# mapbox/robosat

Hardware: NVIDIA H100
Metric: 512x512 tiles/sec (predict fwd) (higher is better)
Workload: dtype f16 hi+lo operand pairs (3 MMAs per K step), fp32 accumulate: strict precision, meets the parity contract

## Files before the change

robosat_b200/csrc/rsb_conv.cu:

```cuda

#include <stdio.h>
#include <string.h>

#include <new>

#include "../../include/rsb200.h"
#include "rsb_host.h"
#include "rsb_ptx.cuh"

namespace rsb {

static constexpr int kBlockM = 128;
static constexpr int kBlockK = 64;
static constexpr int kABytes = kBlockM * kBlockK * 2;
static constexpr int kWgRows = 64;

struct alignas(64) ConvKParams {
    CUtensorMap tmA[RSB_MAX_SRCS];
    CUtensorMap tmB;
    CUtensorMap tmC[4];
    CUtensorMap tmR;
    int32_t nseg;
    int32_t seg_src[RSB_MAX_SEGS];
    int32_t seg_dh[RSB_MAX_SEGS];
    int32_t seg_dw[RSB_MAX_SEGS];
    int32_t seg_cb[RSB_MAX_SEGS];
    int32_t kblocks;
    int32_t tiles_w, tiles_h, tiles_n, n_blocks, phases, total_tiles;
    int32_t pair_tiles;
    int32_t TW, TH, TN;
    int32_t Wt, Ht, Nt;
    int32_t Cout;
    int32_t out_sy, out_sx;
    int64_t out_pitch_w, out_pitch_h, out_pitch_n;
    __half* out;
    const __half* residual;
    const float* bias;
    int32_t relu;
    int32_t head_classes;
    const float* head_w;
    const float* head_b;
    float* head_out;
    float acc_scale;
    float* stats;
    int32_t kchunk;
    float* scratch;
};

template <int BLOCK_N, int MODE, bool HAS_RES, bool TWO = false, int SPLIT = 0>
struct ConvCfg {
    static_assert(SPLIT != 2 || (BLOCK_N <= 64 && !TWO), "the N-concatenated split schedule is for narrow single-CTA tiles");
    static constexpr int kAccN = SPLIT == 2 ? 2 * BLOCK_N : BLOCK_N;
    static constexpr int kPlanes = SPLIT ? 2 : 1;
    static constexpr int kBBytes = BLOCK_N * kBlockK * 2;
    static constexpr int kBHalf = kBBytes / 2;
    static constexpr int kStageA = kPlanes * kABytes;
    static constexpr int kStageB = kPlanes * kBBytes;
    static constexpr int kStageBytes = kStageA + kStageB;
    static constexpr int kChunk = BLOCK_N >= 64 ? 64 : 32;
    static constexpr int kNumChunks = BLOCK_N / kChunk;
    static constexpr int kThreads = 384;
    static constexpr int kWgChunkBytes = kWgRows * kChunk * 2;
    static constexpr int kSliceBytes = kPlanes * kWgChunkBytes;
    static constexpr int kStoreBufs = SPLIT ? 1 : 2;
    static constexpr int kResBufs = HAS_RES ? 2 : 0;
    static constexpr int kEpiBytes = MODE == 0 ? (kStoreBufs + kResBufs) * 2 * kSliceBytes : 0;
    static constexpr int kBarBytes = 512;
    static constexpr int kMaxSmem = 232448;
    static constexpr int kAvail = kMaxSmem - 1024 - kBarBytes - kEpiBytes;
    static constexpr int kStages = (kAvail / kStageBytes) > 8 ? 8 : (kAvail / kStageBytes);
    static_assert(kStages >= 2, "pipeline too shallow");
    static constexpr int kSmemBytes = kStages * kStageBytes + kEpiBytes + kBarBytes + 1024;
};

struct TileCoord {
    int n_blk, pa, pb, phase, w0, h0, n0;
};

__device__ __forceinline__ TileCoord decode_tile(const ConvKParams& p, int id) {
    TileCoord t;
    t.n_blk = id % p.n_blocks;
    id /= p.n_blocks;
    t.phase = id % p.phases;
    id /= p.phases;
    t.pa = t.phase >> 1;
    t.pb = t.phase & 1;
    t.w0 = (id % p.tiles_w) * p.TW;
    id /= p.tiles_w;
    t.h0 = (id % p.tiles_h) * p.TH;
    id /= p.tiles_h;
    t.n0 = id * p.TN;
    return t;
}

template <bool TWO>
__device__ __forceinline__ int item_tile(const ConvKParams& p, int it, int rank) {
    if (!TWO) return it;
    const int per = p.n_blocks * p.phases;
    return ((it / per) * 2 + rank) * per + it % per;
}

__device__ __forceinline__ bool row_valid(const ConvKParams& p, const TileCoord& t, int row) {
    const int w = t.w0 + row % p.TW, h = t.h0 + (row / p.TW) % p.TH, n = t.n0 + row / (p.TW * p.TH);
    return (w < p.Wt) && (h < p.Ht) && (n < p.Nt);
}

template <int BLOCK_N, int MODE, bool HAS_RES, bool TWO, int SPLIT, bool STATS = false>
__global__ void __launch_bounds__(384, 1) conv_tc_kernel(const __grid_constant__ ConvKParams p) {
    using Cfg = ConvCfg<BLOCK_N, MODE, HAS_RES, TWO, SPLIT>;
    const int rank = TWO ? static_cast<int>(cluster_ctarank()) : 0;
    const int item0 = TWO ? static_cast<int>(blockIdx.x >> 1) : static_cast<int>(blockIdx.x);
    const int item_step = TWO ? static_cast<int>(gridDim.x >> 1) : static_cast<int>(gridDim.x);
    const int num_items = TWO ? p.pair_tiles : p.total_tiles;
    extern __shared__ uint8_t smem_raw[];
    uint8_t* smem = reinterpret_cast<uint8_t*>((reinterpret_cast<uintptr_t>(smem_raw) + 1023) & ~uintptr_t(1023));
    uint8_t* smem_a = smem;
    uint8_t* smem_b = smem + Cfg::kStages * Cfg::kStageA;
    uint8_t* smem_c = smem + Cfg::kStages * Cfg::kStageBytes;
    uint8_t* smem_r = smem_c + Cfg::kStoreBufs * 2 * Cfg::kSliceBytes;
    uint64_t* full_bar = reinterpret_cast<uint64_t*>(smem + Cfg::kStages * Cfg::kStageBytes + Cfg::kEpiBytes);
    uint64_t* empty_bar = full_bar + Cfg::kStages;
    uint64_t* res_full_bar = empty_bar + Cfg::kStages;

    const int warp_idx = threadIdx.x >> 5;
    const int lane = threadIdx.x & 31;

    if (warp_idx == 8 && lane == 0) {
        for (int i = 0; i < RSB_MAX_SRCS; ++i) tma_prefetch_desc(&p.tmA[i]);
        tma_prefetch_desc(&p.tmB);
        for (int i = 0; i < Cfg::kStages; ++i) {
            mbar_init(&full_bar[i], 1);
            mbar_init(&empty_bar[i], (TWO ? 2 : 1) * 8);
        }
        for (int i = 0; i < 4; ++i) mbar_init(&res_full_bar[i], 1);
        if (MODE == 0) {
            for (int i = 0; i < 4; ++i) tma_prefetch_desc(&p.tmC[i]);
            if (HAS_RES) tma_prefetch_desc(&p.tmR);
        }
        mbar_fence_init();
    }
    if (TWO) cluster_sync_all();
    else __syncthreads();

    asm volatile("griddepcontrol.launch_dependents;" ::: "memory");
    asm volatile("griddepcontrol.wait;" ::: "memory");

    if (warp_idx >= 8) {
        setmaxnreg_dec<40>();
        if (warp_idx == 8 && elect_one()) {
            int stage = 0;
            uint32_t phase = 0;
            for (int it = item0; it < num_items; it += item_step) {
                const TileCoord t = decode_tile(p, item_tile<TWO>(p, it, rank));
                const int b_row = t.phase * p.Cout + t.n_blk * BLOCK_N;
                int kb = 0;
                for (int s = 0; s < p.nseg; ++s) {
                    const CUtensorMap* tm = &p.tmA[p.seg_src[s]];
                    const int cw = t.w0 + p.seg_dw[s] + t.pb;
                    const int ch = t.h0 + p.seg_dh[s] + t.pa;
                    for (int cb = 0; cb < p.seg_cb[s]; ++cb, ++kb) {
                        mbar_wait(&empty_bar[stage], phase ^ 1);
                        mbar_expect_tx(&full_bar[stage], Cfg::kStageBytes);
                        uint8_t* sa = smem_a + stage * Cfg::kStageA;
                        uint8_t* sb = smem_b + stage * Cfg::kStageB;
                        if constexpr (SPLIT) {
                            tma_load_5d(sa, tm, &full_bar[stage], cb * kBlockK, cw, ch, t.n0, 0);
                        } else {
                            tma_load_4d(sa, tm, &full_bar[stage], cb * kBlockK, cw, ch, t.n0);
                        }
                        if constexpr (TWO) {
                            const int hrow = b_row + rank * (BLOCK_N / 2);
                            if constexpr (SPLIT) {
                                tma_load_3d_mc(sb + rank * Cfg::kBHalf, &p.tmB, &full_bar[stage], kb * kBlockK, hrow, 0, 3);
                                tma_load_3d_mc(sb + Cfg::kBBytes + rank * Cfg::kBHalf, &p.tmB, &full_bar[stage], kb * kBlockK, hrow, 1, 3);
                            } else {
                                tma_load_2d_mc(sb + rank * Cfg::kBHalf, &p.tmB, &full_bar[stage], kb * kBlockK, hrow, 3);
                            }
                        } else if constexpr (SPLIT) {
                            tma_load_3d(sb, &p.tmB, &full_bar[stage], kb * kBlockK, b_row, 0);
                        } else {
                            tma_load_2d(sb, &p.tmB, &full_bar[stage], kb * kBlockK, b_row);
                        }
                        if (++stage == Cfg::kStages) {
                            stage = 0;
                            phase ^= 1;
                        }
                    }
                }
            }
        }
    } else {
        setmaxnreg_inc<232>();
        const int g = warp_idx >> 2;
        const int wtid = threadIdx.x & 127;
        const int r0 = 16 * (warp_idx & 3) + (lane >> 2);
        const int cq = 2 * (lane & 3);
        const int qrow0 = g * kWgRows;
        const int qw = qrow0 % p.TW, qh = (qrow0 / p.TW) % p.TH, qn = qrow0 / (p.TW * p.TH);
        uint8_t* my_c = smem_c + g * Cfg::kStoreBufs * Cfg::kSliceBytes;
        uint8_t* my_r = smem_r + g * (Cfg::kResBufs > 0 ? Cfg::kResBufs : 1) * Cfg::kSliceBytes;
        uint64_t* my_res_bar = res_full_bar + g * 2;
        const uint32_t peer_empty0 = TWO ? mapa_u32(smem_u32(&empty_bar[0]), rank ^ 1) : 0;
        auto release_stage = [&](int s) {
            __syncwarp();
            if (lane == 0) {
                mbar_arrive(&empty_bar[s]);
                if (TWO) mbar_arrive_remote(peer_empty0 + s * 8);
            }
        };
        uint32_t wchunk = 0;
        int res_item = item0;
        int res_chunk = 0;
        auto issue_residual = [&](int rb) {
            if (res_item < num_items) {
                const TileCoord rt = decode_tile(p, item_tile<TWO>(p, res_item, rank));
                mbar_expect_tx(&my_res_bar[rb], Cfg::kSliceBytes);
                if constexpr (SPLIT)
                    tma_load_5d(my_r + rb * Cfg::kSliceBytes, &p.tmR, &my_res_bar[rb], rt.n_blk * BLOCK_N + res_chunk * Cfg::kChunk,
                                rt.w0 + qw, rt.h0 + qh, rt.n0 + qn, 0);
                else
                    tma_load_4d(my_r + rb * Cfg::kSliceBytes, &p.tmR, &my_res_bar[rb], rt.n_blk * BLOCK_N + res_chunk * Cfg::kChunk,
                                rt.w0 + qw, rt.h0 + qh, rt.n0 + qn);
                if (++res_chunk == Cfg::kNumChunks) {
                    res_chunk = 0;
                    res_item += item_step;
                }
            }
        };
        if (MODE == 0 && HAS_RES && wtid == 0) {
#pragma unroll 1
            for (int i = 0; i < Cfg::kResBufs; ++i) issue_residual(i);
        }
        const uint64_t da0 = make_sw128_kmajor_desc(smem_u32(smem_a + g * kWgRows * 128));
        const uint64_t db0 = make_sw128_kmajor_desc(smem_u32(smem_b));
        int stage = 0;
        uint32_t phase = 0;
        const int kchunk = p.kchunk > 0 ? p.kchunk : p.kblocks;
        const int nchunks = (p.kblocks + kchunk - 1) / kchunk;
        float acc[Cfg::kAccN / 2];

        for (int it = item0; it < num_items; it += item_step) {
            const TileCoord t = decode_tile(p, item_tile<TWO>(p, it, rank));
            float* srow0 = p.scratch + (static_cast<size_t>(blockIdx.x) * kBlockM + qrow0 + r0) * BLOCK_N;
            for (int chk = 0; chk < nchunks; ++chk) {
                const int kb0 = chk * kchunk;
                const int kb1 = kb0 + kchunk < p.kblocks ? kb0 + kchunk : p.kblocks;
                int prev = -1;
                for (int kb = kb0; kb < kb1; ++kb) {
                    mbar_wait(&full_bar[stage], phase);
                    const uint64_t da = da0 + static_cast<uint64_t>(stage * (Cfg::kStageA >> 4));
                    const uint64_t db = db0 + static_cast<uint64_t>(stage * (Cfg::kStageB >> 4));
                    acc_fence(acc);
                    wgmma_fence();
#pragma unroll
                    for (int k = 0; k < kBlockK / 16; ++k) {
                        const uint32_t first = (kb != kb0 || k != 0) ? 1u : 0u;
                        if constexpr (SPLIT == 2) {
                            wgmma<2 * BLOCK_N>(acc, da + 2 * k, db + 2 * k, first);
                            wgmma<BLOCK_N, BLOCK_N / 2>(acc, da + (kABytes >> 4) + 2 * k, db + 2 * k, 1u);
                        } else if constexpr (SPLIT == 1) {
                            const uint64_t dal = da + (kABytes >> 4), dbl = db + (Cfg::kBBytes >> 4);
                            wgmma<BLOCK_N>(acc, da + 2 * k, dbl + 2 * k, first);
                            wgmma<BLOCK_N>(acc, dal + 2 * k, db + 2 * k, 1u);
                            wgmma<BLOCK_N>(acc, da + 2 * k, db + 2 * k, 1u);
                        } else {
                            wgmma<BLOCK_N>(acc, da + 2 * k, db + 2 * k, first);
                        }
                    }
                    wgmma_commit();
                    acc_fence(acc);
                    wgmma_wait<1>();
                    if (prev >= 0) release_stage(prev);
                    prev = stage;
                    if (++stage == Cfg::kStages) {
                        stage = 0;
                        phase ^= 1;
                    }
                }
                wgmma_wait<0>();
                acc_fence(acc);
                release_stage(prev);
                if (BLOCK_N <= 128 && nchunks > 1) {
                    const bool last = chk + 1 == nchunks;
#pragma unroll
                    for (int j = 0; j < BLOCK_N / 8; ++j) {
#pragma unroll
                        for (int hh = 0; hh < 2; ++hh) {
                            float* sp = srow0 + hh * 8 * BLOCK_N + 8 * j + cq;
                            const int i = 4 * j + 2 * hh;
                            if constexpr (SPLIT == 2) {
                                acc[i] += acc[BLOCK_N / 2 + i];
                                acc[i + 1] += acc[BLOCK_N / 2 + i + 1];
                                acc[BLOCK_N / 2 + i] = 0.f;
                                acc[BLOCK_N / 2 + i + 1] = 0.f;
                            }
                            if (chk > 0) {
                                const float2 o = *reinterpret_cast<const float2*>(sp);
                                acc[i] += o.x;
                                acc[i + 1] += o.y;
                            }
                            if (!last) *reinterpret_cast<float2*>(sp) = make_float2(acc[i], acc[i + 1]);
                        }
                    }
                }
            }
            auto accv = [&](int j, int hh, int e) {
                float v = acc[4 * j + 2 * hh + e];
                if constexpr (SPLIT == 2) v += acc[BLOCK_N / 2 + 4 * j + 2 * hh + e];
                return v;
            };

            if constexpr (MODE == 0) {
                const float* bptr = p.bias ? p.bias + t.n_blk * BLOCK_N : nullptr;
                const float asc = p.acc_scale;
#pragma unroll
                for (int ck = 0; ck < Cfg::kNumChunks; ++ck, ++wchunk) {
                    constexpr int kRB = Cfg::kResBufs > 0 ? Cfg::kResBufs : 1;
                    const int rb = wchunk % kRB;
                    uint8_t* cbuf = my_c + (wchunk % Cfg::kStoreBufs) * Cfg::kSliceBytes;
                    const uint8_t* rbuf = my_r + rb * Cfg::kSliceBytes;
                    if (wtid == 0) tma_store_wait_read<Cfg::kStoreBufs - 1>();
                    named_bar_sync(1 + g, 128);
                    if (HAS_RES) mbar_wait(&my_res_bar[rb], (wchunk / kRB) & 1);
#pragma unroll
                    for (int jj = 0; jj < Cfg::kChunk / 8; ++jj) {
                        const int j = ck * (Cfg::kChunk / 8) + jj;
                        const int c = 8 * j + cq;
                        float2 b2 = make_float2(0.f, 0.f);
                        if (bptr) b2 = __ldg(reinterpret_cast<const float2*>(bptr + c));
#pragma unroll
                        for (int hh = 0; hh < 2; ++hh) {
                            const int r = r0 + 8 * hh;
                            const int su = Cfg::kChunk == 64 ? (jj ^ (r & 7)) : (jj ^ ((r >> 1) & 3));
                            const int soff = r * (Cfg::kChunk * 2) + su * 16 + (lane & 3) * 4;
                            float a = bptr ? fmaf(accv(j, hh, 0), asc, b2.x) : accv(j, hh, 0) * asc;
                            float b = bptr ? fmaf(accv(j, hh, 1), asc, b2.y) : accv(j, hh, 1) * asc;
                            if (HAS_RES) {
                                const float2 f = __half22float2(*reinterpret_cast<const __half2*>(rbuf + soff));
                                if constexpr (SPLIT) {
                                    const float2 l = __half22float2(*reinterpret_cast<const __half2*>(rbuf + Cfg::kWgChunkBytes + soff));
                                    a += f.x + l.x;
                                    b += f.y + l.y;
                                } else {
                                    a += f.x;
                                    b += f.y;
                                }
                            }
                            if (p.relu) {
                                a = fmaxf(a, 0.0f);
                                b = fmaxf(b, 0.0f);
                            }
                            const __half2 o = __floats2half2_rn(a, b);
                            *reinterpret_cast<__half2*>(cbuf + soff) = o;
                            if constexpr (SPLIT) {
                                const float2 hf = __half22float2(o);
                                *reinterpret_cast<__half2*>(cbuf + Cfg::kWgChunkBytes + soff) = __floats2half2_rn(a - hf.x, b - hf.y);
                            }
                        }
                    }
                    fence_proxy_async_smem();
                    named_bar_sync(1 + g, 128);
                    if constexpr (STATS) {
                        const int hq = warp_idx & 3;
                        if (hq < 2) {
                            const unsigned vmask = __ballot_sync(0xffffffffu, row_valid(p, t, qrow0 + 32 * hq + lane));
                            constexpr int kWords = Cfg::kChunk / 2;
                            constexpr int kGroups = 32 / kWords;
                            const int wd = lane % kWords, gr = lane / kWords;
                            float s0x = 0.f, s0y = 0.f, s1x = 0.f, s1y = 0.f;
#pragma unroll 8
                            for (int r = gr; r < 32; r += kGroups) {
                                const int rr = 32 * hq + r;
                                const int u = wd >> 2;
                                const int su = Cfg::kChunk == 64 ? (u ^ (rr & 7)) : (u ^ ((rr >> 1) & 3));
                                const __half2 hv = *reinterpret_cast<const __half2*>(cbuf + rr * (Cfg::kChunk * 2) + su * 16 + (wd & 3) * 4);
                                if ((vmask >> r) & 1u) {
                                    const float2 f = __half22float2(hv);
                                    s0x += f.x;
                                    s0y += f.y;
                                    s1x = fmaf(f.x, f.x, s1x);
                                    s1y = fmaf(f.y, f.y, s1y);
                                }
                            }
                            if (kGroups == 2) {
                                s0x += __shfl_xor_sync(0xffffffffu, s0x, 16);
                                s0y += __shfl_xor_sync(0xffffffffu, s0y, 16);
                                s1x += __shfl_xor_sync(0xffffffffu, s1x, 16);
                                s1y += __shfl_xor_sync(0xffffffffu, s1y, 16);
                            }
                            const int spatial = item_tile<TWO>(p, it, rank) / p.n_blocks;
                            if (gr == 0 && spatial < p.tiles_w * p.tiles_h * p.tiles_n) {
                                const int q = 2 * g + hq;
                                float* dst = p.stats + (static_cast<size_t>(spatial) * 4 + q) * 2 * p.Cout + t.n_blk * BLOCK_N + ck * Cfg::kChunk + 2 * wd;
                                *reinterpret_cast<float2*>(dst) = make_float2(s0x, s0y);
                                *reinterpret_cast<float2*>(dst + p.Cout) = make_float2(s1x, s1y);
                            }
                        }
                    }
                    if (wtid == 0) {
                        if constexpr (SPLIT)
                            tma_store_5d(&p.tmC[t.phase], cbuf, t.n_blk * BLOCK_N + ck * Cfg::kChunk, t.w0 + qw, t.h0 + qh, t.n0 + qn, 0);
                        else
                            tma_store_4d(&p.tmC[t.phase], cbuf, t.n_blk * BLOCK_N + ck * Cfg::kChunk, t.w0 + qw, t.h0 + qh, t.n0 + qn);
                        tma_store_commit();
                        if (HAS_RES) issue_residual(rb);
                    }
                }
            } else {
                static_assert(MODE == 0 || BLOCK_N == 32, "head mode needs BLOCK_N == 32");
#pragma unroll
                for (int hh = 0; hh < 2; ++hh) {
                    const int row = qrow0 + r0 + 8 * hh;
                    float v[8];
#pragma unroll
                    for (int j = 0; j < 4; ++j) {
#pragma unroll
                        for (int e = 0; e < 2; ++e) {
                            float a = accv(j, hh, e) * p.acc_scale;
                            if (p.bias) a += __ldg(p.bias + 8 * j + cq + e);
                            v[2 * j + e] = p.relu ? fmaxf(a, 0.0f) : a;
                        }
                    }
                    const bool valid = row_valid(p, t, row);
                    const int w = t.w0 + row % p.TW, h = t.h0 + (row / p.TW) % p.TH, n = t.n0 + row / (p.TW * p.TH);
                    for (int k = 0; k < p.head_classes; ++k) {
                        float s = 0.f;
#pragma unroll
                        for (int j = 0; j < 4; ++j) {
                            s = fmaf(__ldg(p.head_w + k * 32 + 8 * j + cq), v[2 * j], s);
                            s = fmaf(__ldg(p.head_w + k * 32 + 8 * j + cq + 1), v[2 * j + 1], s);
                        }
                        s += __shfl_xor_sync(0xffffffffu, s, 1);
                        s += __shfl_xor_sync(0xffffffffu, s, 2);
                        if (valid && (lane & 3) == 0) p.head_out[((static_cast<int64_t>(n) * p.head_classes + k) * p.Ht + h) * p.Wt + w] = s + __ldg(p.head_b + k);
                    }
                }
            }
        }
        if (MODE == 0 && wtid == 0) tma_store_wait<0>();
    }

    if (TWO) cluster_sync_all();
}

__global__ void conv_simt_check_kernel(rsb_conv_desc d, int K) {
    const int64_t total_px = static_cast<int64_t>(d.Nt) * d.Ht * d.Wt * d.phases;
    const int co_per_thread = d.mode == 1 ? d.Cout : 1;
    const int co_threads = d.Cout / co_per_thread;
    const int64_t gid = static_cast<int64_t>(blockIdx.x) * blockDim.x + threadIdx.x;
    if (gid >= total_px * co_threads) return;
    const int co0 = static_cast<int>(gid % co_threads) * co_per_thread;
    int64_t px = gid / co_threads;
    const int phase = static_cast<int>(px % d.phases);
    px /= d.phases;
    const int w = static_cast<int>(px % d.Wt);
    px /= d.Wt;
    const int h = static_cast<int>(px % d.Ht);
    const int n = static_cast<int>(px / d.Ht);
    const int pa = phase >> 1, pb = phase & 1;
    const __half* wts = static_cast<const __half*>(d.weights);
    const int64_t w_plane = static_cast<int64_t>(d.phases) * d.Cout * K;

    float head_acc[8];
    for (int k = 0; k < 8; ++k) head_acc[k] = (d.mode == 1 && k < d.head_classes) ? d.head_b[k] : 0.f;

    for (int co = co0; co < co0 + co_per_thread; ++co) {
        const __half* wrow = wts + (static_cast<int64_t>(phase) * d.Cout + co) * K;
        float acc = 0.f;
        int kidx = 0;
        for (int s = 0; s < d.nseg; ++s) {
            const rsb_conv_src& src = d.srcs[d.segs[s].src];
            const int hh = h + d.segs[s].dh + pa, ww = w + d.segs[s].dw + pb;
            const bool inb = hh >= 0 && hh < src.H && ww >= 0 && ww < src.W && n < src.N;
            const __half* a = static_cast<const __half*>(src.ptr) + n * src.pitch_n + hh * src.pitch_h + ww * src.pitch_w;
            for (int c = 0; c < d.segs[s].cblocks * 64; ++c, ++kidx) {
                if (inb && c < src.C) {
                    float av = __half2float(a[c]), wv = __half2float(wrow[kidx]);
                    if (d.split) {
                        av += __half2float(a[c + src.plane]);
                        wv += __half2float(wrow[kidx + w_plane]);
                    }
                    acc = fmaf(av, wv, acc);
                }
            }
        }
        acc *= d.acc_scale != 0.f ? d.acc_scale : 1.f;
        if (d.bias) acc += d.bias[co];
        const int64_t off = n * d.out_pitch_n + static_cast<int64_t>(h * d.out_sy + pa) * d.out_pitch_h +
                            static_cast<int64_t>(w * d.out_sx + pb) * d.out_pitch_w + co;
        if (d.mode == 0) {
            if (d.residual) {
                float rv = __half2float(static_cast<const __half*>(d.residual)[off]);
                if (d.split) rv += __half2float(static_cast<const __half*>(d.residual)[off + d.res_plane]);
                acc += rv;
            }
            if (d.relu) acc = fmaxf(acc, 0.f);
            const __half hi = __float2half_rn(acc);
            static_cast<__half*>(d.out)[off] = hi;
            if (d.split) static_cast<__half*>(d.out)[off + d.out_plane] = __float2half_rn(acc - __half2float(hi));
        } else {
            if (d.relu) acc = fmaxf(acc, 0.f);
            for (int k = 0; k < d.head_classes; ++k) head_acc[k] = fmaf(d.head_w[k * 32 + co], acc, head_acc[k]);
        }
    }
    if (d.mode == 1) {
        for (int k = 0; k < d.head_classes; ++k)
            d.head_out[((static_cast<int64_t>(n) * d.head_classes + k) * d.Ht + h) * d.Wt + w] = head_acc[k];
    }
}

}

using namespace rsb;

struct rsb_conv_plan {
    ConvKParams kp;
    int block_n;
    int mode;
    int grid;
    int smem;
    bool has_res;
    bool pair;
    bool split;
    bool stats;
};

static int validate_desc(const rsb_conv_desc* d, int* K_out) {
    if (!d) return set_error(RSB_E_INVALID, "conv: null desc");
    if (d->nsrc < 1 || d->nsrc > RSB_MAX_SRCS) return set_error(RSB_E_INVALID, "conv: nsrc out of range");
    if (d->nseg < 1 || d->nseg > RSB_MAX_SEGS) return set_error(RSB_E_INVALID, "conv: nseg out of range");
    if (!(d->block_n == 32 || d->block_n == 64 || d->block_n == 128 || d->block_n == 256))
        return set_error(RSB_E_INVALID, "conv: block_n must be 32/64/128/256");
    if (d->Cout <= 0 || d->Cout % d->block_n) return set_error(RSB_E_INVALID, "conv: Cout not a multiple of block_n");
    if (!(d->phases == 1 || d->phases == 4)) return set_error(RSB_E_INVALID, "conv: phases must be 1 or 4");
    if (d->TW * d->TH * d->TN != kBlockM) return set_error(RSB_E_INVALID, "conv: TW*TH*TN must be 128");
    if (d->Wt <= 0 || d->Ht <= 0 || d->Nt <= 0) return set_error(RSB_E_INVALID, "conv: empty tile space");
    if (!d->weights) return set_error(RSB_E_INVALID, "conv: null weights");
    if (d->split != 0 && d->split != 1) return set_error(RSB_E_INVALID, "conv: split must be 0 or 1");
    int kblocks = 0;
    for (int s = 0; s < d->nseg; ++s) {
        const rsb_conv_seg& g = d->segs[s];
        if (g.src < 0 || g.src >= d->nsrc || g.cblocks < 1) return set_error(RSB_E_INVALID, "conv: bad segment");
        if (g.cblocks * kBlockK > ((d->srcs[g.src].C + kBlockK - 1) / kBlockK) * kBlockK)
            return set_error(RSB_E_INVALID, "conv: segment reads past the source's inner extent");
        kblocks += g.cblocks;
    }
    for (int i = 0; i < d->nsrc; ++i) {
        const rsb_conv_src& s = d->srcs[i];
        if (!s.ptr || (reinterpret_cast<uintptr_t>(s.ptr) & 15)) return set_error(RSB_E_INVALID, "conv: source pointer null or not 16B aligned");
        if ((s.pitch_w * 2) % 16 || (s.pitch_h * 2) % 16 || (s.pitch_n * 2) % 16)
            return set_error(RSB_E_INVALID, "conv: source pitches must be multiples of 16 bytes");
        if (s.C < 1 || s.W < 1 || s.H < 1 || s.N < 1) return set_error(RSB_E_INVALID, "conv: empty source view");
        if (d->split && (s.plane <= 0 || (s.plane * 2) % 16)) return set_error(RSB_E_INVALID, "conv: split needs a positive 16B-multiple plane stride per source");
    }
    if (d->mode == 0) {
        if (!d->out) return set_error(RSB_E_INVALID, "conv: null out");
        if ((reinterpret_cast<uintptr_t>(d->out) & 15) || (d->out_pitch_w * 2) % 16 || (d->out_pitch_h * 2) % 16 ||
            (d->out_pitch_n * 2) % 16)
            return set_error(RSB_E_INVALID, "conv: out must be 16B aligned with 16B-multiple pitches");
        if (d->residual && (reinterpret_cast<uintptr_t>(d->residual) & 15))
            return set_error(RSB_E_INVALID, "conv: residual must be 16B aligned");
        if (d->split && (d->out_plane <= 0 || (d->out_plane * 2) % 16)) return set_error(RSB_E_INVALID, "conv: split needs out_plane");
        if (d->split && d->residual && (d->res_plane <= 0 || (d->res_plane * 2) % 16)) return set_error(RSB_E_INVALID, "conv: split needs res_plane");
        if (d->split && d->residual && d->block_n == 256)
            return set_error(RSB_E_INVALID, "conv: split + residual supports block_n <= 128");
    } else if (d->mode == 1) {
        if (d->block_n != 32 || d->Cout != 32 || d->phases != 1) return set_error(RSB_E_INVALID, "conv: head mode needs Cout == block_n == 32, phases == 1");
        if (d->head_classes < 1 || d->head_classes > 8 || !d->head_w || !d->head_b || !d->head_out)
            return set_error(RSB_E_INVALID, "conv: bad head arguments");
    } else {
        return set_error(RSB_E_INVALID, "conv: unknown mode");
    }
    if (d->cta_pair && (d->mode != 0 || d->block_n < 128)) return set_error(RSB_E_INVALID, "conv: cta_pair needs mode 0 and block_n >= 128");
    if (d->kchunk > 0 && d->block_n > 128) return set_error(RSB_E_INVALID, "conv: kchunk supports block_n <= 128");
    if (d->stats) {
        if (d->mode != 0 || d->split || d->residual || d->phases != 1)
            return set_error(RSB_E_INVALID, "conv: stats needs mode 0, fast precision, no residual, phases == 1");
        const int64_t tiles = static_cast<int64_t>((d->Wt + d->TW - 1) / d->TW) * ((d->Ht + d->TH - 1) / d->TH) * ((d->Nt + d->TN - 1) / d->TN);
        const int64_t need = tiles * 4 * 2 * d->Cout * 4;
        if ((reinterpret_cast<uintptr_t>(d->stats) & 7) || d->stats_bytes < need)
            return set_error(RSB_E_INVALID, "conv: stats needs an 8B-aligned buffer of >= %lld bytes (tiles x 4 x 2 x Cout fp32)", (long long)need);
    }
    *K_out = kblocks * kBlockK;
    return RSB_OK;
}

static constexpr int kMaxDevices = 64;
static int current_device() {
    int dev = 0;
    if (cudaGetDevice(&dev) != cudaSuccess || dev < 0 || dev >= kMaxDevices) dev = 0;
    return dev;
}

template <int BLOCK_N, int MODE, bool HAS_RES, bool TWO, int SPLIT, bool STATS = false>
struct ConvInst {
    using Cfg = ConvCfg<BLOCK_N, MODE, HAS_RES, TWO, SPLIT>;
    static constexpr int kSmem = Cfg::kSmemBytes;

    static int prepare() {
        static bool attr_set[kMaxDevices] = {};
        const int dev = current_device();
        if (!attr_set[dev]) {
            cudaError_t e = cudaFuncSetAttribute(conv_tc_kernel<BLOCK_N, MODE, HAS_RES, TWO, SPLIT, STATS>, cudaFuncAttributeMaxDynamicSharedMemorySize, kSmem);
            if (e != cudaSuccess) return set_cuda_error(e, "cudaFuncSetAttribute(conv)");
            attr_set[dev] = true;
        }
        return RSB_OK;
    }

    static int launch(const rsb_conv_plan* plan, cudaStream_t stream) {
        int rc = prepare();
        if (rc) return rc;
        cudaLaunchConfig_t cfg = {};
        cfg.gridDim = dim3(plan->grid);
        cfg.blockDim = dim3(Cfg::kThreads);
        cfg.dynamicSmemBytes = kSmem;
        cfg.stream = stream;
        cudaLaunchAttribute attr[2];
        attr[0].id = cudaLaunchAttributeProgrammaticStreamSerialization;
        attr[0].val.programmaticStreamSerializationAllowed = 1;
        cfg.attrs = attr;
        cfg.numAttrs = 1;
        if (TWO) {
            attr[1].id = cudaLaunchAttributeClusterDimension;
            attr[1].val.clusterDim.x = 2;
            attr[1].val.clusterDim.y = 1;
            attr[1].val.clusterDim.z = 1;
            cfg.numAttrs = 2;
        }
        cudaError_t e = cudaLaunchKernelEx(&cfg, conv_tc_kernel<BLOCK_N, MODE, HAS_RES, TWO, SPLIT, STATS>, plan->kp);
        if (e != cudaSuccess) return set_cuda_error(e, "conv_tc_kernel launch");
        return RSB_OK;
    }

    static int pair_clusters() {
        static int cached[kMaxDevices];
        static bool have[kMaxDevices] = {};
        const int dev = current_device();
        if (have[dev]) return cached[dev];
        if (prepare() != RSB_OK) return 0;
        cudaLaunchConfig_t cfg = {};
        cfg.gridDim = dim3(2 * num_sms());
        cfg.blockDim = dim3(Cfg::kThreads);
        cfg.dynamicSmemBytes = kSmem;
        cudaLaunchAttribute attr[1];
        attr[0].id = cudaLaunchAttributeClusterDimension;
        attr[0].val.clusterDim.x = 2;
        attr[0].val.clusterDim.y = 1;
        attr[0].val.clusterDim.z = 1;
        cfg.attrs = attr;
        cfg.numAttrs = 1;
        int n = 0;
        if (cudaOccupancyMaxActiveClusters(&n, conv_tc_kernel<BLOCK_N, MODE, HAS_RES, TWO, SPLIT, STATS>, &cfg) != cudaSuccess) {
            cudaGetLastError();
            n = 0;
        }
        const int cap = num_sms() / 2;
        cached[dev] = n < cap ? n : cap;
        have[dev] = true;
        return cached[dev];
    }
};

enum ConvAction { kLaunch, kSmemOf, kPairClusters };

template <int BLOCK_N, int MODE, bool HAS_RES, bool TWO, int SPLIT, bool STATS = false>
static int conv_act(ConvAction a, const rsb_conv_plan* plan, cudaStream_t stream) {
    using I = ConvInst<BLOCK_N, MODE, HAS_RES, TWO, SPLIT, STATS>;
    switch (a) {
        case kLaunch: return I::launch(plan, stream);
        case kSmemOf: return I::kSmem;
        default: return I::pair_clusters();
    }
}

template <int SPLIT>
static int conv_dispatch(ConvAction a, const rsb_conv_plan* plan, cudaStream_t stream) {
    constexpr int NARROW = SPLIT ? 2 : 0;
    if (plan->mode == 1) return conv_act<32, 1, false, false, NARROW>(a, plan, stream);
    if (plan->pair) {
        if (plan->block_n == 128) return plan->has_res ? conv_act<128, 0, true, true, SPLIT>(a, plan, stream) : conv_act<128, 0, false, true, SPLIT>(a, plan, stream);
        if (!plan->has_res) return conv_act<256, 0, false, true, SPLIT>(a, plan, stream);
        if constexpr (!SPLIT) return conv_act<256, 0, true, true, 0>(a, plan, stream);
        return a == kLaunch ? set_error(RSB_E_INVALID, "conv: unsupported block_n / residual / split combination") : 0;
    }
    if (plan->has_res) {
        switch (plan->block_n) {
            case 32: return conv_act<32, 0, true, false, NARROW>(a, plan, stream);
            case 64: return conv_act<64, 0, true, false, NARROW>(a, plan, stream);
            case 128: return conv_act<128, 0, true, false, SPLIT>(a, plan, stream);
            case 256:
                if constexpr (!SPLIT) return conv_act<256, 0, true, false, 0>(a, plan, stream);
                break;
        }
    } else {
        switch (plan->block_n) {
            case 32: return conv_act<32, 0, false, false, NARROW>(a, plan, stream);
            case 64: return conv_act<64, 0, false, false, NARROW>(a, plan, stream);
            case 128: return conv_act<128, 0, false, false, SPLIT>(a, plan, stream);
            case 256: return conv_act<256, 0, false, false, SPLIT>(a, plan, stream);
        }
    }
    return a == kLaunch ? set_error(RSB_E_INVALID, "conv: unsupported block_n / residual / split combination") : 0;
}

static int conv_dispatch_stats(ConvAction a, const rsb_conv_plan* plan, cudaStream_t stream) {
    if (plan->pair) {
        if (plan->block_n == 128) return conv_act<128, 0, false, true, 0, true>(a, plan, stream);
        return conv_act<256, 0, false, true, 0, true>(a, plan, stream);
    }
    switch (plan->block_n) {
        case 32: return conv_act<32, 0, false, false, 0, true>(a, plan, stream);
        case 64: return conv_act<64, 0, false, false, 0, true>(a, plan, stream);
        case 128: return conv_act<128, 0, false, false, 0, true>(a, plan, stream);
        default: return conv_act<256, 0, false, false, 0, true>(a, plan, stream);
    }
}

static int conv_select(ConvAction a, const rsb_conv_plan* plan, cudaStream_t stream) {
    if (plan->stats) return conv_dispatch_stats(a, plan, stream);
    return plan->split ? conv_dispatch<1>(a, plan, stream) : conv_dispatch<0>(a, plan, stream);
}

extern "C" int rsb_conv_plan_create(const rsb_conv_desc* d, rsb_conv_plan** out_plan) {
    if (!out_plan) return set_error(RSB_E_INVALID, "conv: null out_plan");
    *out_plan = nullptr;
    int K = 0;
    int rc = validate_desc(d, &K);
    if (rc) return rc;
    rc = rsb_device_ok();
    if (rc) return rc;

    rsb_conv_plan* plan = new (std::nothrow) rsb_conv_plan();
    if (!plan) return set_error(RSB_E_INVALID, "conv: out of host memory");
    memset(&plan->kp, 0, sizeof(plan->kp));
    ConvKParams& kp = plan->kp;
    const bool split = d->split != 0;
    const int xr = split ? 1 : 0;

    for (int i = 0; i < d->nsrc; ++i) {
        const rsb_conv_src& s = d->srcs[i];
        const uint64_t dims[5] = {(uint64_t)s.C, (uint64_t)s.W, (uint64_t)s.H, (uint64_t)s.N, 2};
        const uint64_t strides[4] = {(uint64_t)s.pitch_w * 2, (uint64_t)s.pitch_h * 2, (uint64_t)s.pitch_n * 2, (uint64_t)s.plane * 2};
        const uint32_t box[5] = {(uint32_t)kBlockK, (uint32_t)d->TW, (uint32_t)d->TH, (uint32_t)d->TN, 2};
        rc = encode_tiled_f16(&kp.tmA[i], 4 + xr, s.ptr, dims, strides, box);
        if (rc) {
            delete plan;
            return rc;
        }
    }
    for (int i = d->nsrc; i < RSB_MAX_SRCS; ++i) kp.tmA[i] = kp.tmA[0];
    {
        const uint64_t rows = (uint64_t)d->phases * d->Cout;
        const uint64_t dims[3] = {(uint64_t)K, rows, 2};
        const uint64_t strides[2] = {(uint64_t)K * 2, rows * (uint64_t)K * 2};
        const uint32_t box[3] = {(uint32_t)kBlockK, (uint32_t)(d->cta_pair ? d->block_n / 2 : d->block_n), d->cta_pair ? 1u : 2u};
        rc = encode_tiled_f16(&kp.tmB, 2 + xr, d->weights, dims, strides, box);
        if (rc) {
            delete plan;
            return rc;
        }
    }
    if (d->mode == 0) {
        const int sy = d->out_sy > 0 ? d->out_sy : 1, sx = d->out_sx > 0 ? d->out_sx : 1;
        const int chunk = d->block_n >= 64 ? 64 : 32;
        const uint64_t dims[5] = {(uint64_t)d->Cout, (uint64_t)d->Wt, (uint64_t)d->Ht, (uint64_t)d->Nt, 2};
        uint64_t strides[4] = {(uint64_t)sx * d->out_pitch_w * 2, (uint64_t)sy * d->out_pitch_h * 2, (uint64_t)d->out_pitch_n * 2,
                               (uint64_t)d->out_plane * 2};
        if (kWgRows % d->TW && d->TW % kWgRows) {
            delete plan;
            return set_error(RSB_E_INVALID, "conv: TW must divide or be a multiple of 64");
        }
        const int bw = d->TW < kWgRows ? d->TW : kWgRows;
        const int bh = (kWgRows / bw) < d->TH ? (kWgRows / bw) : d->TH;
        const int bn = kWgRows / (bw * bh);
        const uint32_t box[5] = {(uint32_t)chunk, (uint32_t)bw, (uint32_t)bh, (uint32_t)bn, 2};
        for (int ph = 0; ph < 4; ++ph) {
            const int a = ph >> 1, b = ph & 1;
            const __half* base = static_cast<const __half*>(d->out) + (ph < d->phases ? a * d->out_pitch_h + b * d->out_pitch_w : 0);
            rc = encode_tiled_f16(&kp.tmC[ph], 4 + xr, base, dims, strides, box, chunk * 2);
            if (rc) {
                delete plan;
                return rc;
            }
        }
        if (d->residual) {
            if (d->phases != 1) {
                delete plan;
                return set_error(RSB_E_INVALID, "conv: residual needs phases == 1");
            }
            strides[3] = (uint64_t)d->res_plane * 2;
            rc = encode_tiled_f16(&kp.tmR, 4 + xr, d->residual, dims, strides, box, chunk * 2);
            if (rc) {
                delete plan;
                return rc;
            }
        } else {
            kp.tmR = kp.tmC[0];
        }
    } else {
        for (int ph = 0; ph < 4; ++ph) kp.tmC[ph] = kp.tmA[0];
        kp.tmR = kp.tmA[0];
    }
    kp.nseg = d->nseg;
    for (int s = 0; s < d->nseg; ++s) {
        kp.seg_src[s] = d->segs[s].src;
        kp.seg_dh[s] = d->segs[s].dh;
        kp.seg_dw[s] = d->segs[s].dw;
        kp.seg_cb[s] = d->segs[s].cblocks;
    }
    kp.kblocks = K / kBlockK;
    kp.TW = d->TW;
    kp.TH = d->TH;
    kp.TN = d->TN;
    kp.Wt = d->Wt;
    kp.Ht = d->Ht;
    kp.Nt = d->Nt;
    kp.tiles_w = (d->Wt + d->TW - 1) / d->TW;
    kp.tiles_h = (d->Ht + d->TH - 1) / d->TH;
    kp.tiles_n = (d->Nt + d->TN - 1) / d->TN;
    kp.n_blocks = d->Cout / d->block_n;
    kp.phases = d->phases;
    kp.total_tiles = kp.tiles_w * kp.tiles_h * kp.tiles_n * kp.n_blocks * kp.phases;
    kp.pair_tiles = ((kp.tiles_w * kp.tiles_h * kp.tiles_n + 1) / 2) * kp.n_blocks * kp.phases;
    kp.Cout = d->Cout;
    kp.out_sy = d->out_sy > 0 ? d->out_sy : 1;
    kp.out_sx = d->out_sx > 0 ? d->out_sx : 1;
    kp.out_pitch_w = d->out_pitch_w;
    kp.out_pitch_h = d->out_pitch_h;
    kp.out_pitch_n = d->out_pitch_n;
    kp.out = static_cast<__half*>(d->out);
    kp.residual = static_cast<const __half*>(d->residual);
    kp.bias = d->bias;
    kp.relu = d->relu;
    kp.head_classes = d->head_classes;
    kp.head_w = d->head_w;
    kp.head_b = d->head_b;
    kp.head_out = d->head_out;
    kp.acc_scale = d->acc_scale != 0.f ? d->acc_scale : 1.f;
    kp.kchunk = (d->kchunk > 0 && d->kchunk < kp.kblocks) ? d->kchunk : 0;
    kp.scratch = d->scratch;
    kp.stats = d->stats;

    plan->block_n = d->block_n;
    plan->mode = d->mode;
    plan->split = split;
    plan->stats = d->stats != nullptr;
    const int sms = num_sms();
    plan->grid = kp.total_tiles < sms ? kp.total_tiles : sms;
    plan->has_res = d->mode == 0 && d->residual != nullptr;
    plan->pair = d->cta_pair != 0;
    if (plan->pair) {
// ... 53 lines not shown
```

robosat_b200/engine.py:

```python

import ctypes
import math
import os
from collections import OrderedDict

import torch

from robosat_b200 import _lib
from robosat_b200._lib import ConvDesc, ConvSeg, ConvSrc, RowConvDesc

RESNET50_BLOCKS = (3, 4, 6, 3)
BN_EPS = 1e-5
IMAGENET_MEAN = (0.485, 0.456, 0.406)
IMAGENET_STD = (0.229, 0.224, 0.225)


def _strip(sd):
    if any(k.startswith("module.") for k in sd):
        return {k[len("module."):]: v for k, v in sd.items()}
    return dict(sd)


def fold_bn(sd, conv_key, bn_prefix):
    w = sd[conv_key].double()
# ... 75 lines not shown
                best = (key, (tw, th, tn))
    return best[1]


CTA_PAIR = os.environ.get("RSB_CTA_PAIR", "1") == "1"


def choose_block_n(cout, m_tiles, phases, kblocks=8, sms=132, split=False):
    cands = [bn for bn in ((128, 64, 32) if split else (256, 128, 64, 32)) if cout % bn == 0]
    assert cands, "Cout must be a multiple of 32"

    def cost(bn):
        tiles = m_tiles * phases * (cout // bn)
        if split:
            mma = 8 * 66 if bn <= 64 else 12 * max(66, bn // 2)
            per_tile = max(kblocks * mma, bn * 28) + 300
        else:
            per_tile = max(kblocks * 4 * max(66, bn // 2), bn * (16 if bn >= 128 else 28)) + 300
        return -(-tiles // sms) * per_tile

    return min(cands, key=lambda bn: (cost(bn), -bn))


class ConvOp:

    def __init__(self, name, desc, keep, create_plan=True):
        self.name = name
        self.desc = desc
        self.keep = keep
        self.plan = ctypes.c_void_p()
        if create_plan:
            lib = _lib.load()
            _lib.check(lib.rsb_conv_plan_create(ctypes.byref(desc), ctypes.byref(self.plan)), "rsb_conv_plan_create[%s]" % name)

    def run(self, stream):
        _lib.check(_lib.load().rsb_conv_run(self.plan, stream), "rsb_conv_run[%s]" % self.name)

    def info(self):
        g, t, k, s = (ctypes.c_int32() for _ in range(4))
        _lib.check(_lib.load().rsb_conv_plan_info(self.plan, ctypes.byref(g), ctypes.byref(t), ctypes.byref(k), ctypes.byref(s)), "plan_info")
        return {"grid": g.value, "tiles": t.value, "kblocks": k.value, "smem": s.value}

    def __del__(self):
        try:
            if self.plan:
                _lib.load().rsb_conv_plan_destroy(self.plan)
                self.plan = ctypes.c_void_p()
        except Exception:
            pass


class RowConvOp:

    def __init__(self, name, desc, keep=(), create_plan=True):
        self.name, self.desc, self.keep = name, desc, keep
        self.plan = ctypes.c_void_p()
        if create_plan:
            _lib.check(_lib.load().rsb_rowconv_plan_create(ctypes.byref(desc), ctypes.byref(self.plan)), "rsb_rowconv_plan_create[%s]" % name)

    def run(self, stream):
        _lib.check(_lib.load().rsb_rowconv_run(self.plan, stream), "rsb_rowconv_run[%s]" % self.name)

    def info(self):
        return {"grid": 0, "tiles": -(-self.desc.Wt // 128) * self.desc.Ht * self.desc.Nt * self.desc.nsub * self.desc.nphase_a, "kblocks": 0, "smem": 0}

    def __del__(self):
        try:
            if self.plan:
                _lib.load().rsb_rowconv_plan_destroy(self.plan)
                self.plan = ctypes.c_void_p()
        except Exception:
            pass


def make_rowconv_desc(src, cin, weights, bias, cout, tile_space, out, out_pitches, upsample=False, relu=True, head=None,
                      out_offset_elems=0, rows_per_unit=0, split=False, acc_scale=1.0):
    d = RowConvDesc()
    d.src = src
    d.cin = cin
    d.taps_h = d.taps_w = 2 if upsample else 3
    d.dh0 = d.dw0 = -1
    d.nsub = d.nphase_a = 2 if upsample else 1
    phases = 4 if upsample else 1
    d.split = 1 if split else 0
    d.acc_scale = acc_scale
    wshape = (phases * cout, d.taps_h * d.taps_w * cin)
    assert weights.dtype == torch.float16 and tuple(weights.shape) == ((2,) + wshape if split else wshape), tuple(weights.shape)
    d.weights = weights.data_ptr()
    d.bias = bias.data_ptr() if bias is not None else None
    d.Cout = cout
    d.Wt, d.Ht, d.Nt = tile_space
    d.relu = 1 if relu else 0
    d.rows_per_unit = rows_per_unit
    if head is None:
        d.mode = 0
        d.out = out.data_ptr() + 2 * out_offset_elems
        d.out_pitch_w, d.out_pitch_h, d.out_pitch_n = out_pitches
        d.out_sy = d.out_sx = 2 if upsample else 1
    else:
        head_w, head_b, head_out, classes = head
        d.mode = 1
        d.head_classes = classes
        d.head_w, d.head_b, d.head_out = head_w.data_ptr(), head_b.data_ptr(), head_out.data_ptr()
    return d


def _src_dense(t, N, H, W, C, plane=0):
    return ConvSrc(t.data_ptr(), C, W * C, H * W * C, C, W, H, N, plane)


def _src_parity(t, N, H, W, C, ph, pw, plane=0):
    return ConvSrc(t.data_ptr() + 2 * (ph * W + pw) * C, 2 * C, 2 * W * C, H * W * C, C, W // 2, H // 2, N, plane)


def make_conv_desc(srcs, segs, weights, bias, cout, phases, tile_space, out, out_pitches, out_scale=(1, 1),
                   residual=None, relu=True, block_n=None, head=None, out_offset_elems=0, cta_pair=None,
                   split=False, acc_scale=1.0, out_plane=0, res_plane=0, scratch=None):
    d = ConvDesc()
    d.split = 1 if split else 0
    d.acc_scale = acc_scale
    d.out_plane = out_plane
    d.res_plane = res_plane
    d.nsrc = len(srcs)
    for i, s in enumerate(srcs):
        d.srcs[i] = s
    d.nseg = len(segs)
    for i, (src, dh, dw, cb) in enumerate(segs):
        d.segs[i] = ConvSeg(src, dh, dw, cb)
    K = 64 * sum(s[3] for s in segs)
    assert weights.dtype == torch.float16 and weights.is_contiguous()
    wshape = (2, phases * cout, K) if split else (phases * cout, K)
    assert tuple(weights.shape) == wshape, (tuple(weights.shape), wshape)
    d.weights = weights.data_ptr()
    d.bias = bias.data_ptr() if bias is not None else None
    d.Cout = cout
    d.phases = phases
    Wt, Ht, Nt = tile_space
    d.Wt, d.Ht, d.Nt = Wt, Ht, Nt
    d.TW, d.TH, d.TN = choose_tile(Wt, Ht, Nt)
    m_tiles = -(-Wt // d.TW) * -(-Ht // d.TH) * -(-Nt // d.TN)
    d.block_n = block_n or choose_block_n(cout, m_tiles, phases, K // 64, split=split)
    if residual is not None and block_n is None and d.block_n == 256:
        d.block_n = 128
    d.out_sy, d.out_sx = out_scale
    d.relu = 1 if relu else 0
    if head is None:
        d.mode = 0
        d.out = out.data_ptr() + 2 * out_offset_elems
        d.out_pitch_w, d.out_pitch_h, d.out_pitch_n = out_pitches
        d.residual = residual.data_ptr() if residual is not None else None
        if cta_pair is None:
            kblocks = K // 64
            if split:
                cta_pair = CTA_PAIR and m_tiles >= 2 and d.block_n >= 128 and kblocks >= 4
            else:
                cta_pair = CTA_PAIR and m_tiles >= 2 and ((d.block_n == 256 and kblocks >= 6) or (d.block_n == 128 and kblocks >= 18))
        d.cta_pair = 1 if cta_pair else 0
        if split and scratch is not None:
            kblocks = K // 64
            per_kb = 12 if d.block_n >= 128 else 4
            if MAX_MMA_CHAIN > 0 and kblocks * per_kb > 2 * MAX_MMA_CHAIN - MAX_MMA_CHAIN // 2:
                nchunks = -(-kblocks * per_kb // MAX_MMA_CHAIN)
                d.kchunk = -(-kblocks // nchunks)
                d.scratch = scratch.data_ptr()
                d.scratch_bytes = scratch.numel() * scratch.element_size()
    else:
        head_w, head_b, head_out, classes = head
        d.mode = 1
        d.head_classes = classes
        d.head_w = head_w.data_ptr()
        d.head_b = head_b.data_ptr()
        d.head_out = head_out.data_ptr()
    return d


PRECISIONS = ("strict", "fast")
MAX_MMA_CHAIN = int(os.environ.get("RSB_MAX_MMA_CHAIN", "400"))


def default_precision():
    p = os.environ.get("RSB_PRECISION", "strict").lower()
    if p not in PRECISIONS:
        raise ValueError("RSB_PRECISION must be one of %s" % (PRECISIONS,))
    return p


_PLAN_TABLE = None


def plan_table():
    global _PLAN_TABLE
    if _PLAN_TABLE is None:
        path = os.environ.get("RSB_PLAN_TABLE", os.path.join(os.path.dirname(os.path.abspath(__file__)), "plans_h100.json"))
        table = {}
        if path not in ("0", "") and os.path.exists(path):
            import json

            with open(path) as fp:
                table = json.load(fp).get("plans", {})
        _PLAN_TABLE = table
    return _PLAN_TABLE


def _override_valid(ov, cout, tile_space, split, has_res):
    bn, pair = int(ov.get("block_n", 0)), bool(ov.get("cta_pair", 0))
    if bn not in (32, 64, 128, 256) or cout % bn:
        return False
    Wt, Ht, Nt = tile_space
    TW, TH, TN = choose_tile(Wt, Ht, Nt)
    m_tiles = -(-Wt // TW) * -(-Ht // TH) * -(-Nt // TN)
    if pair and (bn < 128 or m_tiles < 2 or not CTA_PAIR):
        return False
    if split and bn == 256:
        return False
    return True


class UNetEngine:

    def __init__(self, state_dict, num_classes, batch, height, width, device="cuda", plan_only=False, use_row=True, precision=None,
                 plan_overrides=None):
        assert height % 32 == 0 and width % 32 == 0, "image resolution has to be divisible by 32 for resnet"
        assert height % 64 == 0 and width % 64 == 0, "enc4 must have even extents (input divisible by 64), as in the reference"
        self.plan_only = plan_only
        self.precision = precision or default_precision()
        assert self.precision in PRECISIONS, self.precision
        self.strict = self.precision == "strict"
        self._overrides = plan_overrides if plan_overrides is not None else plan_table().get(
            "%s:%dx%dx%d" % (self.precision, batch, height, width), {})
        self.use_row_head = use_row
        self.use_row = use_row and not self.strict
        if not plan_only:
            _lib.require_device()
        self.device = torch.device(device)
        self.N, self.H, self.W, self.C = batch, height, width, num_classes
        self.ops = []
        self.feats = OrderedDict()
        self._keep = []
        where = torch.device("cpu") if plan_only else self.device
        self._build({k: v.detach().to(where) for k, v in _strip(state_dict).items()})

    def _buf(self, *shape, dtype=torch.float16):
        t = torch.zeros(shape, dtype=dtype, device=self.device)
        self._keep.append(t)
        return t

    def _act(self, *shape):
        return self._buf(*((2,) + shape if self.strict else shape))

    def _plane(self, t):
        return t.numel() // 2 if self.strict else 0

    def _dev(self, t, dtype):
        t = t.to(dtype).contiguous().to(self.device)
        self._keep.append(t)
        return t

    def _wts(self, w):
        if not self.strict:
            return self._dev(w, torch.float16), 1.0
        hi, lo, scale = split_fp16(w)
        return self._dev(torch.stack([hi, lo]), torch.float16), scale

    def _scratch(self):
        if getattr(self, "_scratch_buf", None) is None:
            n = 132 * 128 * 256 if self.plan_only else int(_lib.load().rsb_conv_scratch_bytes(256)) // 4
            self._scratch_buf = self._buf(n, dtype=torch.float32)
        return self._scratch_buf

    def _dense(self, t, N, H, W, C):
        return _src_dense(t, N, H, W, C, self._plane(t))

    def _parity(self, t, N, H, W, C, ph, pw):
        return _src_parity(t, N, H, W, C, ph, pw, self._plane(t))

    def _conv(self, name, srcs, segs, w, b, cout, phases, tile_space, out, out_pitches, residual=None, **kw):
        wd, scale = self._wts(w)
        bd = self._dev(b, torch.float32) if b is not None else None

        def build(extra):
            desc = make_conv_desc(srcs, segs, wd, bd, cout, phases, tile_space, out, out_pitches, residual=residual,
                                  split=self.strict, acc_scale=scale, out_plane=self._plane(out) if out is not None else 0,
                                  res_plane=self._plane(residual) if residual is not None else 0,
                                  scratch=self._scratch() if self.strict else None, **dict(kw, **extra))
            return ConvOp(name, desc, (wd, bd), create_plan=not self.plan_only)

        op = None
        ov = self._overrides.get(name)
        if ov and "block_n" not in kw and "cta_pair" not in kw and "head" not in kw and _override_valid(ov, cout, tile_space, self.strict, residual is not None):
            try:
                op = build({"block_n": int(ov["block_n"]), "cta_pair": bool(ov["cta_pair"])})
            except _lib.RsbError:
                op = None
        if op is None:
            op = build({})
        self.ops.append(("conv", op))
        return op

    def _add_row(self, name, desc):
        op = RowConvOp(name, desc, (), create_plan=not self.plan_only)
        self.ops.append(("conv", op))
        return op

    def _build(self, sd):
        N, H, W = self.N, self.H, self.W
        H2, W2 = H // 2, W // 2
        dev = self._dev

        self.s2d = self._act(N, H2, W2 + 4, 16)
        self.ops.append(("prepass",))

        w, b = fold_bn(sd, "resnet.conv1.weight", "resnet.bn1")
        stem = self._act(N, H2, W2, 64)
        Wp = W2 + 4
        src = ConvSrc(self.s2d.data_ptr(), 16, Wp * 16, H2 * Wp * 16, 64, W2, H2, N, self._plane(self.s2d))
        segs = [(0, t - 2, 0, 1) for t in range(4)]
        self._conv("stem", [src], segs, pack_stem(w), b, 64, 1, (W2, H2, N), stem, (64, W2 * 64, H2 * W2 * 64))
        self.feats["stem"] = (stem, (N, H2, W2, 64))

        H4, W4 = H // 4, W // 4
        enc0 = self._act(N, H4, W4, 64)
        self.ops.append(("maxpool", stem, enc0, N, H2, W2, 64, 3, 2, 1))
        self.feats["enc0"] = (enc0, (N, H4, W4, 64))

        cur, curC, curH, curW = enc0, 64, H4, W4
        encs = []
        for li, blocks in enumerate(RESNET50_BLOCKS, start=1):
            planes = 64 * 2 ** (li - 1)
            for bi in range(blocks):
                p = "resnet.layer%d.%d" % (li, bi)
                stride = 2 if (bi == 0 and li > 1) else 1
                oH, oW = curH // stride, curW // stride
                w, b = fold_bn(sd, p + ".conv1.weight", p + ".bn1")
                t1 = self._act(N, curH, curW, planes)
                self._conv(p + ".conv1", [self._dense(cur, N, curH, curW, curC)], [(0, 0, 0, curC // 64)], pack_conv(w), b,
                           planes, 1, (curW, curH, N), t1, (planes, curW * planes, curH * curW * planes))
                w, b = fold_bn(sd, p + ".conv2.weight", p + ".bn2")
                t2 = self._act(N, oH, oW, planes)
                if stride == 1 and planes == 64 and self.use_row and curW >= 128:
                    self._add_row(p + ".conv2", make_rowconv_desc(_src_dense(t1, N, curH, curW, planes), planes, dev(pack_conv(w), torch.float16),
                                                                  dev(b, torch.float32), planes, (oW, oH, N), t2, (planes, oW * planes, oH * oW * planes)))
                    srcs = None
                elif stride == 1:
                    srcs = [self._dense(t1, N, curH, curW, planes)]
                    segs = [(0, kh - 1, kw - 1, planes // 64) for kh in range(3) for kw in range(3)]
                else:
                    srcs = [self._parity(t1, N, curH, curW, planes, ph, pw) for ph in range(2) for pw in range(2)]
                    segs = []
                    for kh in range(3):
                        for kw in range(3):
                            ph, dh = (kh - 1) % 2, (kh - 1) // 2
                            pw, dw = (kw - 1) % 2, (kw - 1) // 2
                            segs.append((ph * 2 + pw, dh, dw, planes // 64))
                if srcs is not None:
                    self._conv(p + ".conv2", srcs, segs, pack_conv(w), b, planes, 1, (oW, oH, N), t2, (planes, oW * planes, oH * oW * planes))
                outC = planes * 4
                w3, b3 = fold_bn(sd, p + ".conv3.weight", p + ".bn3")
                out = self._act(N, oH, oW, outC)
                t2src = self._dense(t2, N, oH, oW, planes)
                if (p + ".downsample.0.weight") in sd:
                    wd, bd = fold_bn(sd, p + ".downsample.0.weight", p + ".downsample.1")
                    xsrc = self._dense(cur, N, curH, curW, curC) if stride == 1 else self._parity(cur, N, curH, curW, curC, 0, 0)
                    wcat = torch.cat([pack_conv(w3), pack_conv(wd)], dim=1)
                    self._conv(p + ".conv3+downsample", [t2src, xsrc], [(0, 0, 0, planes // 64), (1, 0, 0, curC // 64)], wcat, b3 + bd,
                               outC, 1, (oW, oH, N), out, (outC, oW * outC, oH * oW * outC))
                else:
# ... 115 lines not shown
```

Before: 1236.

## Use split main/cross accumulators for strict 128-wide single-CTA conv tiles

Extends the SPLIT==2 schedule to 128-wide tiles. The two cross-term MMAs (hi*lo, lo*hi) now go into a separate accumulator half, which is summed into the main accumulator once per chunk rather than in the epilogue. The engine also stops picking CTA pairs in strict mode and disables K-chunking for those tiles, which should shorten the dependent MMA chain and avoid scratch round-trips. In exchange the 128-wide tiles hold twice the accumulator registers and lose the paired-CTA schedule, so register pressure rises.

```diff
diff --git a/robosat_b200/csrc/rsb_conv.cu b/robosat_b200/csrc/rsb_conv.cu
--- a/robosat_b200/csrc/rsb_conv.cu
+++ b/robosat_b200/csrc/rsb_conv.cu
@@ -49,8 +49,9 @@
 
 template <int BLOCK_N, int MODE, bool HAS_RES, bool TWO = false, int SPLIT = 0>
 struct ConvCfg {
-    static_assert(SPLIT != 2 || (BLOCK_N <= 64 && !TWO), "the N-concatenated split schedule is for narrow single-CTA tiles");
+    static_assert(SPLIT != 2 || (BLOCK_N <= 128 && !TWO), "the [main | cross] split schedule is for single-CTA tiles up to 128 columns");
     static constexpr int kAccN = SPLIT == 2 ? 2 * BLOCK_N : BLOCK_N;
+    static constexpr bool kChunked = !(SPLIT == 2 && BLOCK_N == 128);
     static constexpr int kPlanes = SPLIT ? 2 : 1;
     static constexpr int kBBytes = BLOCK_N * kBlockK * 2;
     static constexpr int kBHalf = kBBytes / 2;
@@ -235,11 +236,15 @@
         const uint64_t db0 = make_sw128_kmajor_desc(smem_u32(smem_b));
         int stage = 0;
         uint32_t phase = 0;
-        const int kchunk = p.kchunk > 0 ? p.kchunk : p.kblocks;
-        const int nchunks = (p.kblocks + kchunk - 1) / kchunk;
+        const int kchunk = Cfg::kChunked && p.kchunk > 0 ? p.kchunk : p.kblocks;
+        const int nchunks = Cfg::kChunked ? (p.kblocks + kchunk - 1) / kchunk : 1;
         float acc[Cfg::kAccN / 2];
 
         for (int it = item0; it < num_items; it += item_step) {
+            if constexpr (SPLIT == 2) {
+#pragma unroll
+                for (int i = 0; i < Cfg::kAccN / 2; ++i) acc[i] = 0.f;
+            }
             const TileCoord t = decode_tile(p, item_tile<TWO>(p, it, rank));
             float* srow0 = p.scratch + (static_cast<size_t>(blockIdx.x) * kBlockM + qrow0 + r0) * BLOCK_N;
             for (int chk = 0; chk < nchunks; ++chk) {
@@ -255,7 +260,12 @@
 #pragma unroll
                     for (int k = 0; k < kBlockK / 16; ++k) {
                         const uint32_t first = (kb != kb0 || k != 0) ? 1u : 0u;
-                        if constexpr (SPLIT == 2) {
+                        if constexpr (SPLIT == 2 && BLOCK_N == 128) {
+                            const uint64_t dal = da + (kABytes >> 4), dbl = db + (Cfg::kBBytes >> 4);
+                            wgmma<BLOCK_N, BLOCK_N / 2>(acc, da + 2 * k, dbl + 2 * k, first);
+                            wgmma<BLOCK_N, BLOCK_N / 2>(acc, dal + 2 * k, db + 2 * k, 1u);
+                            wgmma<BLOCK_N>(acc, da + 2 * k, db + 2 * k, first);
+                        } else if constexpr (SPLIT == 2) {
                             wgmma<2 * BLOCK_N>(acc, da + 2 * k, db + 2 * k, first);
                             wgmma<BLOCK_N, BLOCK_N / 2>(acc, da + (kABytes >> 4) + 2 * k, db + 2 * k, 1u);
                         } else if constexpr (SPLIT == 1) {
@@ -280,7 +290,11 @@
                 wgmma_wait<0>();
                 acc_fence(acc);
                 release_stage(prev);
-                if (BLOCK_N <= 128 && nchunks > 1) {
+                if constexpr (SPLIT == 2) {
+#pragma unroll
+                    for (int i = 0; i < BLOCK_N / 2; ++i) acc[i] += acc[BLOCK_N / 2 + i];
+                }
+                if (BLOCK_N <= 128 && Cfg::kChunked && nchunks > 1) {
                     const bool last = chk + 1 == nchunks;
 #pragma unroll
                     for (int j = 0; j < BLOCK_N / 8; ++j) {
@@ -288,12 +302,6 @@
                         for (int hh = 0; hh < 2; ++hh) {
                             float* sp = srow0 + hh * 8 * BLOCK_N + 8 * j + cq;
                             const int i = 4 * j + 2 * hh;
-                            if constexpr (SPLIT == 2) {
-                                acc[i] += acc[BLOCK_N / 2 + i];
-                                acc[i + 1] += acc[BLOCK_N / 2 + i + 1];
-                                acc[BLOCK_N / 2 + i] = 0.f;
-                                acc[BLOCK_N / 2 + i + 1] = 0.f;
-                            }
                             if (chk > 0) {
                                 const float2 o = *reinterpret_cast<const float2*>(sp);
                                 acc[i] += o.x;
@@ -304,11 +312,7 @@
                     }
                 }
             }
-            auto accv = [&](int j, int hh, int e) {
-                float v = acc[4 * j + 2 * hh + e];
-                if constexpr (SPLIT == 2) v += acc[BLOCK_N / 2 + 4 * j + 2 * hh + e];
-                return v;
-            };
+            auto accv = [&](int j, int hh, int e) { return acc[4 * j + 2 * hh + e]; };
 
             if constexpr (MODE == 0) {
                 const float* bptr = p.bias ? p.bias + t.n_blk * BLOCK_N : nullptr;
@@ -573,6 +577,8 @@
     }
     if (d->cta_pair && (d->mode != 0 || d->block_n < 128)) return set_error(RSB_E_INVALID, "conv: cta_pair needs mode 0 and block_n >= 128");
     if (d->kchunk > 0 && d->block_n > 128) return set_error(RSB_E_INVALID, "conv: kchunk supports block_n <= 128");
+    if (d->kchunk > 0 && d->split && d->block_n == 128 && !d->cta_pair)
+        return set_error(RSB_E_INVALID, "conv: kchunk is not supported by single-CTA strict 128-wide tiles");
     if (d->stats) {
         if (d->mode != 0 || d->split || d->residual || d->phases != 1)
             return set_error(RSB_E_INVALID, "conv: stats needs mode 0, fast precision, no residual, phases == 1");
@@ -676,8 +682,8 @@
 
 template <int SPLIT>
 static int conv_dispatch(ConvAction a, const rsb_conv_plan* plan, cudaStream_t stream) {
-    constexpr int NARROW = SPLIT ? 2 : 0;
-    if (plan->mode == 1) return conv_act<32, 1, false, false, NARROW>(a, plan, stream);
+    constexpr int XACC = SPLIT ? 2 : 0;
+    if (plan->mode == 1) return conv_act<32, 1, false, false, XACC>(a, plan, stream);
     if (plan->pair) {
         if (plan->block_n == 128) return plan->has_res ? conv_act<128, 0, true, true, SPLIT>(a, plan, stream) : conv_act<128, 0, false, true, SPLIT>(a, plan, stream);
         if (!plan->has_res) return conv_act<256, 0, false, true, SPLIT>(a, plan, stream);
@@ -686,18 +692,18 @@
     }
     if (plan->has_res) {
         switch (plan->block_n) {
-            case 32: return conv_act<32, 0, true, false, NARROW>(a, plan, stream);
-            case 64: return conv_act<64, 0, true, false, NARROW>(a, plan, stream);
-            case 128: return conv_act<128, 0, true, false, SPLIT>(a, plan, stream);
+            case 32: return conv_act<32, 0, true, false, XACC>(a, plan, stream);
+            case 64: return conv_act<64, 0, true, false, XACC>(a, plan, stream);
+            case 128: return conv_act<128, 0, true, false, XACC>(a, plan, stream);
             case 256:
                 if constexpr (!SPLIT) return conv_act<256, 0, true, false, 0>(a, plan, stream);
                 break;
         }
     } else {
         switch (plan->block_n) {
-            case 32: return conv_act<32, 0, false, false, NARROW>(a, plan, stream);
-            case 64: return conv_act<64, 0, false, false, NARROW>(a, plan, stream);
-            case 128: return conv_act<128, 0, false, false, SPLIT>(a, plan, stream);
+            case 32: return conv_act<32, 0, false, false, XACC>(a, plan, stream);
+            case 64: return conv_act<64, 0, false, false, XACC>(a, plan, stream);
+            case 128: return conv_act<128, 0, false, false, XACC>(a, plan, stream);
             case 256: return conv_act<256, 0, false, false, SPLIT>(a, plan, stream);
         }
     }
diff --git a/robosat_b200/engine.py b/robosat_b200/engine.py
--- a/robosat_b200/engine.py
+++ b/robosat_b200/engine.py
@@ -251,14 +251,15 @@
         if cta_pair is None:
             kblocks = K // 64
             if split:
-                cta_pair = CTA_PAIR and m_tiles >= 2 and d.block_n >= 128 and kblocks >= 4
+                cta_pair = False
             else:
                 cta_pair = CTA_PAIR and m_tiles >= 2 and ((d.block_n == 256 and kblocks >= 6) or (d.block_n == 128 and kblocks >= 18))
         d.cta_pair = 1 if cta_pair else 0
         if split and scratch is not None:
             kblocks = K // 64
-            per_kb = 12 if d.block_n >= 128 else 4
-            if MAX_MMA_CHAIN > 0 and kblocks * per_kb > 2 * MAX_MMA_CHAIN - MAX_MMA_CHAIN // 2:
+            per_kb = 4 if not d.cta_pair and d.block_n <= 128 else 12
+            chunkable = d.block_n < 128 or (d.block_n == 128 and d.cta_pair)
+            if chunkable and MAX_MMA_CHAIN > 0 and kblocks * per_kb > 2 * MAX_MMA_CHAIN - MAX_MMA_CHAIN // 2:
                 nchunks = -(-kblocks * per_kb // MAX_MMA_CHAIN)
                 d.kchunk = -(-kblocks // nchunks)
                 d.scratch = scratch.data_ptr()
@@ -311,6 +312,8 @@
     if pair and (bn < 128 or m_tiles < 2 or not CTA_PAIR):
         return False
     if split and bn == 256:
+        return False
+    if split and pair:
         return False
     return True
 
```

New measurement: 1257 (median of 6 runs). 1.02x the previous value.
